# jungmannlab/picasso

Measured on AMD Instinct MI355X. Metric: localizations/sec (7x7 ROI, MLE), higher is better.
Workload: dtype f32+f64; 1 GPU; 10000-frame 512x512 uint16 simulated DNA-PAINT movie per GPU, 1001675 spots per GPU, 7x7 ROI MLE (sigmaxy), identify+cut+fit+table resident in HBM; frames=10000, height=512, width=512, box=7, max_it=100, localizations_total=1001675, mle_mode=refit, refit_spots_rank0=7346, frame_ranges_in_flight=2, all_gather=none

## Files before the change

### picasso_amd/csrc/fit_common.h

```cpp
#pragma once
#include <math.h>

#include "pmi_common.h"

namespace pmi {

#ifndef FIT_WAVES_N
#define FIT_WAVES_N 4
#endif
constexpr int FIT_WAVES = FIT_WAVES_N;
constexpr int FIT_NT = FIT_WAVES * PMI_WAVE;
constexpr int FIT_MAXPIX = PMI_MAX_BOX * PMI_MAX_BOX;

struct ConstDiv { float g, r; int fast; };
inline ConstDiv make_const_div(float g)
{
    ConstDiv c;
    c.g = g;
    c.r = (float)(1.0 / (double)g);
    c.fast = (g == g) && fabsf(g) > 1e-15f && fabsf(g) < 1e15f;
    if (g == 1.0f) c.fast = 2;
    return c;
}
__device__ __forceinline__ float div_const(float x, const ConstDiv &c)
{
    if (c.fast == 2) return x;
    const float ax = fabsf(x);
    if (!c.fast || !((ax > 1e-15f && ax < 1e15f) || x == 0.0f)) return x / c.g;
    const float q = x * c.r;
    const float e = __builtin_fmaf(-q, c.g, x);
    return __builtin_fmaf(e, c.r, q);
}
template <int B> __device__ __forceinline__ void div_const_row(float (&v)[B], const ConstDiv &c)
{
    if (c.fast == 2) return;
    unsigned hi = 0u, lo = 0xffffffffu;
#pragma unroll
    for (int i = 0; i < B; i++) {
        const unsigned u = __float_as_uint(v[i]) & 0x7fffffffu;
        hi = u > hi ? u : hi;
        const unsigned w = u - 1u;
        lo = w < lo ? w : lo;
    }
    if (c.fast && hi < 0x58635fa9u && lo >= 0x26901d7du) {
#pragma unroll
        for (int i = 0; i < B; i++) {
            const float q = v[i] * c.r;
            const float e = __builtin_fmaf(-q, c.g, v[i]);
            v[i] = __builtin_fmaf(e, c.r, q);
        }
    } else {
#pragma unroll
        for (int i = 0; i < B; i++) v[i] = v[i] / c.g;
    }
}

struct FitParams {
    const float *spots;
    float *spots_out;
    const void *movie;
    const int32_t *frame, *y, *x;
    int dtype;
    int64_t Y, X;
    float baseline, sensitivity, gain;
    ConstDiv gdiv;
    int64_t N;
    const int64_t *d_n;
    int box;
    int libm_glibc;
    double eps;
    int max_it;
    float *thetas, *crlbs, *loglik;
    int32_t *iterations;
    unsigned long long *queue;
    unsigned *strict_queue;
    int64_t first;
    double *fisher;
    float eps_lo, eps_hi;
    int32_t *flag_list;
    unsigned *flag_count;
    unsigned *flag_reasons;
    const int32_t *final_list;
    const unsigned *final_list_n;
    unsigned char *refit_mark;
    float *ng_io;
    unsigned char *accept;
    int crop_y0, crop_x0, crop_cy, crop_cx;
    double min_ng;
    const int32_t *alist;
    const unsigned *alist_n;
    int32_t *alist_out;
    unsigned *alist_blk_out;
};
enum : unsigned { FLAG_MARGIN = 1u, FLAG_CURVATURE = 2u, FLAG_NARROW = 4u, FLAG_SWING = 8u, FLAG_WILD = 16u, FLAG_SLOW = 32u, FLAG_UNSTABLE = 64u };
constexpr int FLAG_REASONS = 7;
constexpr double FIT_UNSTABLE_LMAX = 1.9;
constexpr int FISHER_STRIDE = 21;
enum { FIT_STAGE_NEWTON = 1, FIT_STAGE_FINAL = 2, FIT_STAGE_INIT_ONLY = 4, FIT_STAGE_ITERATE_ONLY = 8 };
constexpr int FIT_SLOW_ITERATIONS = 64;
#ifndef PMI_MARGIN_GROWTH
#define PMI_MARGIN_GROWTH 0.0625f
#endif
constexpr float FIT_MARGIN_GROWTH = PMI_MARGIN_GROWTH;
constexpr float FIT_NARROW_SIGMA = 0.5f;
constexpr float FIT_WOBBLE_RATIO = 0.9f;
constexpr float FIT_WOBBLE_FLOOR = 1.9073486e-6f;
constexpr int FIT_WOBBLE_RUN = 3;
constexpr int FIT_WOBBLE_LATE = 9;
constexpr float FIT_TOP_FLAG = 16.0f;

template <int CTRL, int ROW_MASK = 0xf>
__device__ __forceinline__ float dpp_f(float v)
// ... 96 lines not shown
```

### picasso_amd/csrc/gaussmle.hip

```cpp
#include <algorithm>
#include <cmath>
#include <cstdlib>
#include <cstring>
#include <vector>

#include "fit_common.h"

namespace pmi {

__device__ __forceinline__ unsigned borderline(float D, int kk, float eps_lo, float eps_hi)
{
    const float wide = fmaxf(1.0f, (float)(kk - 1) * FIT_MARGIN_GROWTH);
    const float epsf = 0.5f * (eps_lo + eps_hi), epsm = 0.5f * (eps_hi - eps_lo) * wide;
    return ((D >= epsf - epsm && D < epsf + epsm) ? FLAG_MARGIN : 0u) | (kk > FIT_SLOW_ITERATIONS ? FLAG_SLOW : 0u);
}
struct StepHistory { float prev, prev2, wprev; int run; };
__device__ __forceinline__ bool wobbles(float st, float value, int kk, StepHistory &h)
{
    const float w = kk >= 3 ? (st - 2.0f * h.prev) + h.prev2 : 0.0f;
    const bool wob = w * h.wprev < 0.0f && fabsf(w) > FIT_WOBBLE_RATIO * fabsf(h.wprev) && fabsf(w) > FIT_WOBBLE_FLOOR * fabsf(value);
    h.run = wob ? h.run + 1 : 0;
    h.wprev = w; h.prev2 = h.prev; h.prev = st;
    return h.run >= FIT_WOBBLE_RUN || (h.run >= 2 && kk >= FIT_WOBBLE_LATE);
}
// ... 562 lines not shown
        if (!strcmp(env, "glibc")) return PMI_LIBM_GLIBC;
        if (!strcmp(env, "device")) return PMI_LIBM_DEVICE;
    }
    return g_mle_libm;
}

int fit_impl(FitParams p, int method, bool from_movie, int range, hipStream_t s)
{
    if (p.box < 3 || p.box > PMI_MAX_BOX || (p.box & 1) == 0) { set_error("box must be odd, 3..%d (got %d)", PMI_MAX_BOX, p.box); return PMI_ERR_ARG; }
    if (method != PMI_MLE_SIGMA && method != PMI_MLE_SIGMAXY) { set_error("Method not available."); return PMI_ERR_ARG; }
    if (p.N < 0) { set_error("negative N"); return PMI_ERR_ARG; }
    if (p.N == 0) return PMI_OK;
    if (p.N > 0x7fffffffLL) { set_error("too many spots for one call"); return PMI_ERR_ARG; }
    const int g_cu_count = device_cu_count();
    const int mode = mle_mode_now();
    const int64_t BATCH = FIT_BATCH;
    const int64_t nb = (p.N + BATCH - 1) / BATCH;
    void *ptr = nullptr, *fptr = nullptr;
    int rc;
    if ((rc = scratch(SCR_FIT, (size_t)nb * 40 + 64, &ptr)) != PMI_OK) return rc;
    const size_t per_batch = (size_t)std::min<int64_t>(p.N, BATCH);
    const size_t acc_blocks = (per_batch + ACC_BLOCK - 1) / ACC_BLOCK + 2;
    if ((rc = scratch(SCR_STAGE_D, per_batch * (FISHER_STRIDE * sizeof(double) + 12 * sizeof(float) + 3 * sizeof(int32_t) + 1) + acc_blocks * sizeof(unsigned) + 32, &fptr)) != PMI_OK) return rc;
    float *state = reinterpret_cast<float *>((char *)fptr + per_batch * FISHER_STRIDE * sizeof(double));
    int32_t *flag_list = reinterpret_cast<int32_t *>(state + per_batch * 12);
    int32_t *unstable_list = flag_list + per_batch;
    int32_t *acc_list = unstable_list + per_batch;
    unsigned *acc_blk = reinterpret_cast<unsigned *>(acc_list + per_batch);
    unsigned char *refit_mark = reinterpret_cast<unsigned char *>(acc_blk + acc_blocks);
    unsigned long long *queues = (unsigned long long *)ptr;
    unsigned *flag_counts = (unsigned *)(queues + 3 * nb);
    unsigned *strict_queues = flag_counts + 2 * nb;
    void *sptr = nullptr;
    if ((rc = scratch(SCR_STATS, 64, &sptr)) != PMI_OK) return rc;
    unsigned *stats = (unsigned *)sptr;
    hipLaunchKernelGGL(zero_words_kernel, dim3(1), dim3(256), 0, s, (unsigned *)ptr, (int)(nb * 10), stats, 16);
    p.flag_reasons = stats + 1;
    p.fisher = (double *)fptr;
    const int libm = mle_libm_now();
    const bool libm_all = libm != PMI_LIBM_DEVICE;
    p.libm_glibc = libm == PMI_LIBM_GLIBC || (libm == PMI_LIBM_AUTO && p.box <= 5);
    static const char *menv = tuning_env("PMI_MLE_MARGIN");
    const double margin = menv ? atof(menv) : g_mle_margin;
    const double ulp = ldexp(1.0, (int)floor(log2(std::max(1.0, p.box / 2.0))) - 23);
    const double margin_abs = std::max(p.eps * margin, 4.0 * ulp);
    p.eps_lo = (float)(p.eps - margin_abs);
    p.eps_hi = (float)(p.eps + margin_abs);
    const int ppl = (p.box * p.box + 63) / 64;
    const int64_t Ntotal = p.N;
    ScopedKernelTimer tm(s, &g_last_times.fit_ms);
    static const bool force_wave_per_spot = tuning_env("PMI_FIT_WAVE_PER_SPOT") != nullptr;
    const bool g8 = !force_wave_per_spot && p.box <= 15;
    float *cut = nullptr;
    static const bool no_keep = tuning_env("PMI_MLE_NO_KEEP") != nullptr;
    if (g8 && from_movie && mode != PMI_MLE_STRICT && !no_keep) {
        void *cptr = nullptr;
        if ((rc = scratch(SCR_STAGE_C, per_batch * (size_t)(p.box * p.box) * sizeof(float), &cptr)) != PMI_OK) return rc;
        cut = (float *)cptr;
    }
    p.spots_out = nullptr;
    if (p.ng_io && !(g8 && from_movie && cut)) { set_error("deferred exact stage outside the row-per-lane fit"); return PMI_ERR_ARG; }
    for (int64_t bi = 0; bi < nb; bi++) {
        p.first = bi * BATCH;
        p.N = std::min<int64_t>(Ntotal, p.first + BATCH);
        p.flag_list = mode == PMI_MLE_REFIT ? flag_list : nullptr;
        p.flag_count = flag_counts + bi;
        p.strict_queue = strict_queues + bi;
        p.refit_mark = mode == PMI_MLE_REFIT ? refit_mark : nullptr;
        if (p.refit_mark && !g8) PMI_HIP(hipMemsetAsync(refit_mark, 0, (size_t)(p.N - p.first), s));
        const int64_t count = p.N - p.first;
        const int64_t blocks = std::min<int64_t>((count + FIT_WAVES - 1) / FIT_WAVES, (int64_t)g_cu_count * 8);
        const dim3 grid((unsigned)std::max<int64_t>(blocks, 1));
        auto wave_per_spot = [&](int stages) {
            p.queue = queues + 3 * bi + (stages == FIT_STAGE_FINAL ? (p.final_list ? 2 : 1) : 0);
            if (method == PMI_MLE_SIGMAXY) {
                if (from_movie) launch_fit_ppl<6, true>(ppl, grid, s, p, stages); else launch_fit_ppl<6, false>(ppl, grid, s, p, stages);
            } else {
                if (from_movie) launch_fit_ppl<5, true>(ppl, grid, s, p, stages); else launch_fit_ppl<5, false>(ppl, grid, s, p, stages);
            }
        };
        if (mode != PMI_MLE_STRICT && g8 && from_movie && cut) {
            FitParams pi = p;
            pi.spots_out = cut;
            launch_fit_g8(pi, method, true, g_cu_count, state, FIT_STAGE_INIT_ONLY, s);
            PMI_HIP(hipGetLastError());
            FitParams q = p;
            q.spots = cut - p.first * (int64_t)(p.box * p.box);
            if (p.ng_io) {
                int32_t *al = nb == 1 && p.alist_out ? p.alist_out : acc_list;
                unsigned *ab = nb == 1 && p.alist_out ? p.alist_blk_out : acc_blk;
                if ((rc = build_accept_list(p.accept, p.first, p.N, p.d_n, ab, al, s)) != PMI_OK) return rc;
                q.alist = al;
                q.alist_n = ab + (count + ACC_BLOCK - 1) / ACC_BLOCK;
            }
            launch_fit_g8(q, method, false, g_cu_count, state, FIT_STAGE_ITERATE_ONLY, s);
            PMI_HIP(hipGetLastError());
            if (mode == PMI_MLE_REFIT)
                launch_fit_strict(q, method, false, flag_list, q.flag_count, count, g_cu_count, s);
            PMI_HIP(hipGetLastError());
            launch_fit_g8(q, method, false, g_cu_count, state, FIT_STAGE_FINAL, s);
        } else {
        if (mode == PMI_MLE_STRICT) {
            FitParams ps = p;
            ps.libm_glibc = libm_all;
            launch_fit_strict(ps, method, from_movie, nullptr, nullptr, count, g_cu_count, s);
        } else {
            if (g8) launch_fit_g8(p, method, from_movie, g_cu_count, state, FIT_STAGE_NEWTON, s);
            else wave_per_spot(FIT_STAGE_NEWTON);
            PMI_HIP(hipGetLastError());
            if (mode == PMI_MLE_REFIT)
                launch_fit_strict(p, method, from_movie, flag_list, p.flag_count, count, g_cu_count, s);
        }
        PMI_HIP(hipGetLastError());
        if (g8) launch_fit_g8(p, method, from_movie, g_cu_count, state, FIT_STAGE_FINAL, s);
        else wave_per_spot(FIT_STAGE_FINAL);
        }
        PMI_HIP(hipGetLastError());
        const unsigned cb = (unsigned)((count + 255) / 256);
        unsigned *unstable_n = flag_counts + nb + bi;
        auto crlb = [&](const int32_t *list, const unsigned *list_n, int32_t *out, unsigned *out_n) {
            if (method == PMI_MLE_SIGMAXY)
                hipLaunchKernelGGL((crlb_kernel<6>), dim3(cb), dim3(256), 0, s, p.fisher, p.first, p.N, p.d_n, p.crlbs, list, list_n, out, out_n, p.flag_reasons, p.refit_mark, p.accept);
            else
                hipLaunchKernelGGL((crlb_kernel<5>), dim3(cb), dim3(256), 0, s, p.fisher, p.first, p.N, p.d_n, p.crlbs, list, list_n, out, out_n, p.flag_reasons, p.refit_mark, p.accept);
        };
        const bool second = mode == PMI_MLE_REFIT;
        crlb(nullptr, nullptr, second ? unstable_list : nullptr, second ? unstable_n : nullptr);
        PMI_HIP(hipGetLastError());
        if (second) {
            FitParams r = p;
            r.strict_queue = strict_queues + nb + bi;
            if (cut) { r.spots = cut - p.first * (int64_t)(p.box * p.box); }
            const bool r_movie = cut ? false : from_movie;
            launch_fit_strict(r, method, r_movie, unstable_list, unstable_n, count, g_cu_count, s);
            PMI_HIP(hipGetLastError());
            r.final_list = unstable_list; r.final_list_n = unstable_n;
            if (g8) launch_fit_g8(r, method, r_movie, g_cu_count, state, FIT_STAGE_FINAL, s);
            else {
                FitParams keep = p;
                p = r;
                wave_per_spot(FIT_STAGE_FINAL);
                p = keep;
            }
            PMI_HIP(hipGetLastError());
            crlb(unstable_list, unstable_n, nullptr, nullptr);
            PMI_HIP(hipGetLastError());
        }
    }
    hipLaunchKernelGGL(flag_stats_kernel, dim3(1), dim3(1), 0, s, flag_counts, mode == PMI_MLE_REFIT ? 2 * nb : 0, stats);
    PMI_HIP(hipGetLastError());
    if ((rc = g_mle_stats.record(0, range, stats, s)) != PMI_OK) return rc;
    tm.stop();
    return PMI_OK;
}

static int read_last_stats(unsigned (&h)[16], hipStream_t s)
{
    if (g_mle_stats.valid()) PMI_HIP(hipStreamSynchronize(s));
    return g_mle_stats.read(h);
}

__global__ void cut_spots_kernel(const void *__restrict__ movie, int dtype, int64_t Y, int64_t X,
                                 const int32_t *__restrict__ frame, const int32_t *__restrict__ y,
                                 const int32_t *__restrict__ x, int64_t N, const int64_t *__restrict__ d_n,
                                 int box, float baseline, float sensitivity, ConstDiv gdiv, float *__restrict__ spots)
{
    int64_t n = N;
    if (d_n) { int64_t dn = *d_n; n = dn < n ? dn : n; }
    const int npix = box * box, h = box / 2;
    int64_t total = n * npix;
    for (int64_t t = (int64_t)blockIdx.x * blockDim.x + threadIdx.x; t < total; t += (int64_t)gridDim.x * blockDim.x) {
        int64_t i = t / npix;
        int q = (int)(t - i * npix);
        int a = q / box, c = q - a * box;
        float raw = load_movie_px(movie, dtype, ((int64_t)frame[i] * Y + (y[i] - h + a)) * X + (x[i] - h + c));
        spots[t] = div_const((raw - baseline) * sensitivity, gdiv);
    }
}

struct LocCols { void *c[PMI_LOC_COLUMNS]; };
__global__ void locs_from_fits_kernel(const int32_t *__restrict__ frame, const int32_t *__restrict__ y,
                                      const int32_t *__restrict__ x, const float *__restrict__ ng,
                                      const float *__restrict__ th, const float *__restrict__ cr,
                                      const float *__restrict__ ll, const int32_t *__restrict__ it, int64_t N,
                                      const int64_t *__restrict__ d_n, int box, LocCols cols, const int64_t *__restrict__ d_row0,
// ... 319 lines not shown
```

### picasso_amd/csrc/gaussmle_g8.hip

```cpp
#include <algorithm>

#include "fit_common.h"
#include "ng_common.h"

namespace pmi {

__device__ __forceinline__ float sum8(float v)
{
    v += dpp_f<0xB1>(v);
    v += dpp_f<0x4E>(v);
    v += dpp_f<0x141>(v);
    return v;
}
__device__ __forceinline__ float min8(float v)
{
    v = fminf(v, dpp_f<0xB1>(v));
    v = fminf(v, dpp_f<0x4E>(v));
    v = fminf(v, dpp_f<0x141>(v));
    return v;
}
__device__ __forceinline__ double sum8_d(double v)
{
    v += dpp_d<0xB1>(v);
    v += dpp_d<0x4E>(v);
// ... 94 lines not shown
    return t;
}

#ifndef G8_PACKED_BOUNDARY
#define G8_PACKED_BOUNDARY 1
#endif
typedef float f32x2 __attribute__((ext_vector_type(2)));
struct BTerms2 { f32x2 E, A, A2, S, S2; };
__device__ __forceinline__ f32x2 splat2(float v) { return (f32x2){v, v}; }
__device__ __forceinline__ f32x2 fma2(f32x2 a, f32x2 b, f32x2 c) { return __builtin_elementwise_fma(a, b, c); }
__device__ __forceinline__ f32x2 erf_f32x2(f32x2 a)
{
    const f32x2 t = {fabsf(a.x), fabsf(a.y)}, s = a * a;
    f32x2 r = fma2(splat2(-1.72853470e-5f), t, splat2(3.83197126e-4f));
    const f32x2 u = fma2(splat2(-3.88396438e-3f), t, splat2(2.42546219e-2f));
    r = fma2(r, s, u);
    r = fma2(r, t, splat2(-1.06777877e-1f));
    r = fma2(r, t, splat2(-6.34846687e-1f));
    r = fma2(r, t, splat2(-1.28717512e-1f));
    r = fma2(r, t, -t);
    const f32x2 ex = {__expf(r.x), __expf(r.y)};
    const f32x2 one_m = splat2(1.0f) - ex;
    const f32x2 big = {copysignf(one_m.x, a.x), copysignf(one_m.y, a.y)};
    f32x2 q = splat2(-5.96761703e-4f);
    q = fma2(q, s, splat2(4.99119423e-3f));
    q = fma2(q, s, splat2(-2.67681349e-2f));
    q = fma2(q, s, splat2(1.12819925e-1f));
    q = fma2(q, s, splat2(-3.76125336e-1f));
    q = fma2(q, s, splat2(1.28379166e-1f));
    const f32x2 small = fma2(q, a, a);
    return (f32x2){t.x > 0.921875f ? big.x : small.x, t.y > 0.921875f ? big.y : small.y};
}
__device__ __forceinline__ BTerms2 boundary_terms2(float jf, f32x2 mu, f32x2 sigma)
{
    const f32x2 is = {rcp_f32(sigma.x), rcp_f32(sigma.y)};
    const f32x2 sn = splat2(0.70710678118654757f) * is, c1 = splat2(0.3989422804014327f) * is, is2 = is * is;
    const f32x2 u0 = splat2(jf - 0.5f) - mu;
    const f32x2 e0 = erf_f32x2(u0 * sn);
    const f32x2 ga = splat2(-0.5f) * u0 * u0 * is2;
    const f32x2 g0 = {__expf(ga.x), __expf(ga.y)};
    const f32x2 e1 = {from_next(e0.x), from_next(e0.y)}, g1 = {from_next(g0.x), from_next(g0.y)};
    const f32x2 u1 = u0 + splat2(1.0f);
    const f32x2 q1 = u0 * g0 - u1 * g1;
    const f32x2 q3 = u0 * u0 * u0 * g0 - u1 * u1 * u1 * g1;
    BTerms2 t;
    t.E = splat2(0.5f) * (e1 - e0);
    t.A = (g0 - g1) * c1;
    t.A2 = q1 * c1 * is2;
    t.S = q1 * c1 * is;
    t.S2 = c1 * is2 * (q3 * is2 - splat2(2.0f) * q1);
    return t;
}

template <int B, bool FROM_MOVIE>
__device__ __forceinline__ void load_row(const FitParams &p, int64_t sidx, int j, bool valid, float (&d)[B])
{
    constexpr int H = B / 2;
#pragma unroll
    for (int i = 0; i < B; i++) d[i] = 0.f;
    if (valid) {
        if (FROM_MOVIE) {
            float raw[B];
            const int64_t fr = p.frame[sidx], yy = p.y[sidx], xx = p.x[sidx];
            const int64_t o = (fr * p.Y + (yy - H + j)) * p.X + (xx - H);
            switch (p.dtype) {
            case PMI_U16: { const uint16_t *q = (const uint16_t *)p.movie + o; _Pragma("unroll") for (int i = 0; i < B; i++) raw[i] = (float)q[i]; } break;
            case PMI_U8:  { const uint8_t *q = (const uint8_t *)p.movie + o;   _Pragma("unroll") for (int i = 0; i < B; i++) raw[i] = (float)q[i]; } break;
            case PMI_I16: { const int16_t *q = (const int16_t *)p.movie + o;   _Pragma("unroll") for (int i = 0; i < B; i++) raw[i] = (float)q[i]; } break;
            case PMI_U32: { const uint32_t *q = (const uint32_t *)p.movie + o; _Pragma("unroll") for (int i = 0; i < B; i++) raw[i] = (float)q[i]; } break;
            case PMI_I32: { const int32_t *q = (const int32_t *)p.movie + o;   _Pragma("unroll") for (int i = 0; i < B; i++) raw[i] = (float)q[i]; } break;
            default:      { const float *q = (const float *)p.movie + o;       _Pragma("unroll") for (int i = 0; i < B; i++) raw[i] = q[i]; } break;
            }
#pragma unroll
            for (int i = 0; i < B; i++)
                d[i] = (raw[i] - p.baseline) * p.sensitivity;
            div_const_row<B>(d, p.gdiv);
        } else {
            const float *sp = p.spots + sidx * (B * B) + j * B;
#pragma unroll
            for (int i = 0; i < B; i++) d[i] = sp[i];
        }
    }
}

#ifndef G8_REFILL_K
#define G8_REFILL_K 2
#endif
template <int GS> struct GLds { static constexpr int N = GS * 12 + GS * 12 + (GS == 8 ? 16 : 16); };

struct LaneRole {
    float ms;
    float floor_, cap;
    float th;
    float prev, prev2;
    float wprev;
    int run;
    bool conv_rel;
};

template <int NP, int B>
__device__ __forceinline__ bool newton_step(const float (&d)[B], float (&th)[6], LaneRole &role, float *lds,
                                            int j, bool rowok, bool active, int &kk, double eps, int max_it,
                                            float eps_lo, float eps_hi, unsigned &flags)
{
    constexpr int GS = GroupOf<B>::GS;
    float *cols = lds, *red = lds + GS * 12, *bc = lds + 2 * GS * 12;
    const float jf = (float)j;
    const float sgy = NP == 6 ? th[5] : th[4];
    BTerms tx, ty;
#if G8_PACKED_BOUNDARY
    {
        const BTerms2 b = boundary_terms2(jf, (f32x2){th[0], th[1]}, (f32x2){th[4], sgy});
        tx.E = b.E.x; tx.A = b.A.x; tx.A2 = b.A2.x; tx.S = b.S.x; tx.S2 = b.S2.x;
        ty.E = b.E.y; ty.A = b.A.y; ty.A2 = b.A2.y; ty.S = b.S.y; ty.S2 = b.S2.y;
    }
#else
    tx = boundary_terms(jf, th[0], th[4]);
    ty = boundary_terms(jf, th[1], sgy);
#endif
    __builtin_amdgcn_wave_barrier();
    {
        float4 *c = reinterpret_cast<float4 *>(cols + j * 12);
        c[0] = make_float4(tx.A, tx.E, tx.S, tx.A2);
        c[1] = make_float4(tx.S2, 1.0f, tx.A * tx.A, tx.E * tx.E);
        c[2] = make_float4(tx.S * tx.S, 1.0f, tx.S * tx.E, 0.0f);
    }
    __builtin_amdgcn_wave_barrier();
    __threadfence_block();

// ... 201 lines not shown
            if (spot_ok && (rowok || edge_lane)) load_nb_row<W>(p.movie, p.dtype, (fr * p.Y + r1) * p.X + (xx - H - 1), c0, nb);
            if (spot_ok && edge_lane) load_nb_row<W>(p.movie, p.dtype, (fr * p.Y + (yy + H + 1)) * p.X + (xx - H - 1), c0, nb2);
#pragma unroll
            for (int i = 0; i < B; i++) d[i] = 0.f;
            if (spot_ok && rowok) {
#pragma unroll
                for (int i = 0; i < B; i++) d[i] = (nb[i + 1] - p.baseline) * p.sensitivity;
                div_const_row<B>(d, p.gdiv);
            }
            loaded = true;
            if (__any(need)) {
                if (rowok) {
#pragma unroll
                    for (int c = 0; c < W; c++) nbt[(j + 1) * W + c] = nb[c];
                }
                if (edge_lane) {
#pragma unroll
                    for (int c = 0; c < W; c++) { nbt[c] = nb[c]; nbt[(W - 1) * W + c] = nb2[c]; }
                }
                __builtin_amdgcn_wave_barrier();
                __threadfence_block();
                const float vc = nbt[(H + 1) * W + (H + 1)];
                bool fm = true;
                if (rowok) {
#pragma unroll
                    for (int l = 0; l < B; l++) {
                        const float o = nb[l + 1];
                        const bool before = j < H || (j == H && l < H);
                        const bool centre = j == H && l == H;
                        fm = fm && (centre || (before ? vc > o : vc >= o));
                        const float gy = sub_rn(nbt[(j + 2) * W + l + 1], nbt[j * W + l + 1]);
                        const float gx = sub_rn(nb[l + 2], nb[l]);
                        terms[j * B + l] = add_rn(mul_rn(gy, uy[l]), mul_rn(gx, ux[l]));
                    }
                }
                __builtin_amdgcn_wave_barrier();
                __threadfence_block();
                float ng = 0.0f;
#pragma unroll
                for (int q = 0; q < B * B; q++)
                    if (q != H * B + H) ng = add_rn(ng, terms[q]);
                const unsigned long long gm = (GS == 64 ? ~0ull : ((1ull << GS) - 1ull)) << (lane & ~(GS - 1));
                const bool first_max = (__ballot(fm) & gm) == gm;
                if (need) {
                    keep = first_max && (double)ng > p.min_ng;
                    if (j == 0) p.ng_io[sidx] = ng;
                }
                __builtin_amdgcn_wave_barrier();
            }
            if (spot_ok && j == 0) p.accept[sidx] = keep ? 1 : 0;
        }
    }
    if (!loaded) load_row<B, FROM_MOVIE>(p, sidx, j, spot_ok && rowok, d);
    if (FROM_MOVIE && p.spots_out && spot_ok && rowok && keep) {
        float *o = p.spots_out + (sidx - p.first) * (B * B) + j * B;
#pragma unroll
        for (int i = 0; i < B; i++) o[i] = d[i];
    }

    double ps = 0.0, px = 0.0;
#pragma unroll
    for (int i = 0; i < B; i++) { ps += (double)d[i]; px += (double)d[i] * (double)i; }
    double sum = gsum_d<GS>(ps), sx_ = gsum_d<GS>(px), sy_ = gsum_d<GS>(ps * (double)j);
    float fmin_l = INFINITY;
    {
        double t3[B];
#pragma unroll
        for (int i = 0; i < B; i++) {
            double a = (double)d[i];
            if (i > 0) a = (double)d[i - 1] + a;
            if (i + 1 < B) a += (double)d[i + 1];
            t3[i] = a;
        }
        const bool up = j > 0, dn = j + 1 < B;
        const int nrow = 1 + (up ? 1 : 0) + (dn ? 1 : 0);
        const double n2 = (double)(nrow * 2), n3 = (double)(nrow * 3);
        const double r2 = 1.0 / n2, r3 = 1.0 / n3;
#pragma unroll
        for (int i = 0; i < B; i++) {
            const double a = from_prev_d(t3[i]), c = from_next_d(t3[i]);
            double tot = t3[i];
            if (up) tot = a + tot;
            if (dn) tot += c;
            const bool edge = (i == 0) || (i + 1 == B);
            const double nn = edge ? n2 : n3, rr = edge ? r2 : r3;
            double q = tot * rr;
            q = fma(fma(-q, nn, tot), rr, q);
            const float filt = (float)q;
            if (rowok) fmin_l = fminf(fmin_l, filt);
        }
    }
    const float bg0 = (sum != sum) ? (float)sum : gmin<GS>(fmin_l);
    double com_y, com_x;
    if (sum <= 0.0) { sum = 0.01; com_y = (B - 1) / 2.0; com_x = (B - 1) / 2.0; }
    else { com_y = sy_ / sum; com_x = sx_ / sum; }
    double photons = sum - (double)(B * B) * (double)bg0;
    photons = (photons != photons) ? photons : (photons > 1.0 ? photons : 1.0);
    double a_sdy = 0.0, a_sy = 0.0, a_sdx = 0.0, a_sx = 0.0;
    if (rowok) {
        const float vm = d[H] - bg0;
        a_sdy = (double)vm * (double)((j - H) * (j - H));
        a_sy = (double)vm;
        if (j == H) {
#pragma unroll
            for (int i = 0; i < B; i++) {
                const float v2 = d[i] - bg0;
                a_sdx += (double)v2 * (double)((i - H) * (i - H));
                a_sx += (double)v2;
            }
        }
    }
    a_sdy = gsum_d<GS>(a_sdy); a_sy = gsum_d<GS>(a_sy); a_sdx = gsum_d<GS>(a_sdx); a_sx = gsum_d<GS>(a_sx);
    double isy = sqrt(a_sdy / a_sy), isx = sqrt(a_sdx / a_sx);
    if (!isfinite(isy)) isy = 0.01;
    if (!isfinite(isx)) isx = 0.01;
    if (isx == 0) isx = 0.01;
    if (isy == 0) isy = 0.01;

    float th[6], ms[6];
    th[0] = (float)com_x; th[1] = (float)com_y; th[2] = (float)photons; th[3] = bg0;
    if (NP == 6) { th[4] = (float)isx; th[5] = (float)isy; }
    else { th[4] = (float)((isx + isy) / 2); th[5] = 0.f; }
    ms[0] = th[4]; ms[1] = th[4];
    ms[2] = (float)(0.1 * (double)th[2]); ms[3] = (float)(0.1 * (double)th[3]);
    ms[4] = (float)(0.2 * (double)th[4]); ms[5] = (float)(0.2 * (double)th[5]);
    if (spot_ok && j == 0) {
        if (p.refit_mark) p.refit_mark[sidx - p.first] = 0;
        float4 *so = reinterpret_cast<float4 *>(state + (sidx - p.first) * 12);
        so[0] = make_float4(th[0], th[1], th[2], th[3]);
        so[1] = make_float4(th[4], th[5], ms[0], ms[1]);
        so[2] = make_float4(ms[2], ms[3], ms[4], ms[5]);
    }
}

template <int NP, int B, bool FROM_MOVIE>
__global__ __launch_bounds__(FIT_NT) void g8_iterate_kernel(FitParams p, const float *__restrict__ state)
{
    constexpr int GS = GroupOf<B>::GS, NSPW = 64 / GS;
    constexpr int REFILL_K = GS == 8 ? G8_REFILL_K : 1;
    __shared__ __attribute__((aligned(16))) float s_x[FIT_WAVES][NSPW][GLds<GS>::N];
    const int lane = threadIdx.x & 63, wid = threadIdx.x >> 6;
    const int g = lane / GS, j = lane & (GS - 1);
    const bool rowok = j < B;
    int64_t n = p.N;
    if (p.d_n) { int64_t dn = *p.d_n; n = dn < n ? dn : n; }
    const int64_t count = p.alist ? (int64_t)*p.alist_n : n - p.first;
    if (count <= 0) return;
    const int64_t total_waves = (int64_t)gridDim.x * FIT_WAVES;
    const int64_t chunk = (count + total_waves - 1) / total_waves;
    const int64_t wv = (int64_t)blockIdx.x * FIT_WAVES + __builtin_amdgcn_readfirstlane(wid);
    const int64_t base = p.alist ? 0 : p.first, lim = base + count;
    int64_t next = base + wv * chunk;
    const int64_t end = next + chunk < lim ? next + chunk : lim;
    if (next >= end) return;

    float *xs = &s_x[wid][g][0];
    float d[B], th[6], ms[6];
#pragma unroll
    for (int i = 0; i < B; i++) d[i] = 1.f;
#pragma unroll
    for (int l = 0; l < 6; l++) { th[l] = 1.f; ms[l] = 1.f; }
    LaneRole role = make_role<NP, B>(th, ms, j);
    int kk = 0;
    int64_t sidx = -1;
    bool active = false;
    unsigned flags = 0u;
    const unsigned long long below = (1ull << (lane & ~(GS - 1))) - 1ull;

    for (;;) {
        const unsigned long long pend = __ballot(!active && sidx >= 0 && j == 0);
        const unsigned long long empty = __ballot(!active && sidx < 0 && j == 0);
        const bool any_active = __any(active);
        if (__popcll(pend) >= REFILL_K || (pend != 0 && !any_active) || (empty != 0 && next < end)) {
            const unsigned gflag = gor_u<GS>(flags);
            if (!active && sidx >= 0 && j == 0) {
                float *to = p.thetas + sidx * 6;
#pragma unroll
                for (int l = 0; l < 5; l++) to[l] = th[l];
                to[5] = NP == 6 ? th[5] : th[4];
                p.iterations[sidx] = kk;
                if (gflag && p.flag_list) {
                    p.flag_list[atomicAdd(p.flag_count, 1u)] = (int32_t)sidx;
                    count_flag_reasons(p.flag_reasons, gflag);
                }
            }
            const unsigned long long want = pend | empty;
            const int64_t cand = next + __popcll(want & below);
            if (!active) {
                sidx = -1;
                if (cand < end) {
                    sidx = p.alist ? (int64_t)p.alist[cand] : cand;
                    const float4 *si = reinterpret_cast<const float4 *>(state + (sidx - p.first) * 12);
                    const float4 s0 = si[0], s1 = si[1], s2 = si[2];
                    th[0] = s0.x; th[1] = s0.y; th[2] = s0.z; th[3] = s0.w; th[4] = s1.x; th[5] = s1.y;
                    ms[0] = s1.z; ms[1] = s1.w; ms[2] = s2.x; ms[3] = s2.y; ms[4] = s2.z; ms[5] = s2.w;
                    load_row<B, FROM_MOVIE>(p, sidx, j, rowok, d);
                    role = make_role<NP, B>(th, ms, j);
                    kk = 0;
                    flags = 0u;
                    active = p.max_it > 0;
                    if (!active && j == 0) {
                        float *to = p.thetas + sidx * 6;
#pragma unroll
                        for (int l = 0; l < 5; l++) to[l] = th[l];
                        to[5] = NP == 6 ? th[5] : th[4];
                        p.iterations[sidx] = 0;
                        sidx = -1;
                    }
                }
            }
            next += __popcll(want);
            if (!__any(active)) {
                if (next >= end) break;
                continue;
            }
        } else if (!any_active) {
            break;
        }
        active = newton_step<NP, B>(d, th, role, xs, j, rowok, active, kk, p.eps, p.max_it, p.eps_lo, p.eps_hi, flags);
    }
}

template <int NP, int B, bool FROM_MOVIE>
__global__ __launch_bounds__(FIT_NT) void g8_final_kernel(FitParams p)
{
    constexpr int GS = GroupOf<B>::GS, NSPW = 64 / GS;
    __shared__ __attribute__((aligned(16))) double s_x[FIT_WAVES][NSPW][GS * 7];
    const int lane = threadIdx.x & 63, wid = threadIdx.x >> 6;
    const int g = lane / GS, j = lane & (GS - 1);
    const bool rowok = j < B;
    const float jf = (float)j;
    int64_t n = p.N;
    if (p.d_n) { int64_t dn = *p.d_n; n = dn < n ? dn : n; }
    int64_t sidx = p.first + ((int64_t)blockIdx.x * FIT_WAVES + wid) * NSPW + g;
    bool spot_ok = sidx < n;
    if (p.final_list) {
        const int64_t w0 = ((int64_t)blockIdx.x * FIT_WAVES + wid) * NSPW, items = (int64_t)*p.final_list_n;
        if (__builtin_amdgcn_readfirstlane((int)(w0 >= items))) return;
        spot_ok = w0 + g < items;
        sidx = spot_ok ? (int64_t)p.final_list[w0 + g] : p.first;
    } else if (__builtin_amdgcn_readfirstlane((int)(p.first + ((int64_t)blockIdx.x * FIT_WAVES + wid) * NSPW >= n))) return;
    else if (p.accept) spot_ok = spot_ok && p.accept[sidx] != 0;

    float d[B], th[6];
    load_row<B, FROM_MOVIE>(p, sidx, j, spot_ok && rowok, d);
#pragma unroll
    for (int l = 0; l < 6; l++) th[l] = spot_ok ? p.thetas[sidx * 6 + l] : 1.f;
    double *red = &s_x[wid][g][0];
    float *cols = reinterpret_cast<float *>(red);
    const float sgy = NP == 6 ? th[5] : th[4];
    const BTerms tx = boundary_terms<true>(jf, th[0], th[4]);
    const BTerms ty = boundary_terms<true>(jf, th[1], sgy);
    {
        float4 *c = reinterpret_cast<float4 *>(cols + j * 12);
        c[0] = make_float4(tx.A * tx.A, tx.A * tx.E, tx.A, tx.A * tx.S);
        c[1] = make_float4(tx.E * tx.E, tx.E, tx.E * tx.S, 1.0f);
        c[2] = make_float4(tx.S, tx.S * tx.S, 0.f, 0.f);
    }
    __builtin_amdgcn_wave_barrier();
    __threadfence_block();
    double T[10];
#pragma unroll
    for (int e = 0; e < 10; e++) T[e] = 0.0;
    float ll_loc = 0.f;
    const float N_ = th[2];
    const float NEy = N_ * ty.E;
#pragma unroll
    for (int i = 0; i < B; i++) {
        const float4 *c = reinterpret_cast<const float4 *>(cols + i * 12);
        const float4 c0 = c[0], c1 = c[1];
        const float2 c2 = *reinterpret_cast<const float2 *>(cols + i * 12 + 8);
        const float model = NEy * c1.y + th[3];
        if (rowok) {
            const double md = (double)model;
            double inv = (double)rcp_f32(model);
            inv = inv * (2.0 - md * inv);
            inv = inv * (2.0 - md * inv);
            T[0] += (double)c0.x * inv; T[1] += (double)c0.y * inv; T[2] += (double)c0.z * inv; T[3] += (double)c0.w * inv;
            T[4] += (double)c1.x * inv; T[5] += (double)c1.y * inv; T[6] += (double)c1.z * inv; T[7] += inv;
            T[8] += (double)c2.x * inv; T[9] += (double)c2.y * inv;
            if (model > 0.f) {
                if (d[i] > 0.f) ll_loc += d[i] * __logf(model / d[i]) - (model - d[i]);
                else ll_loc += -model;
            }
        }
    }
    __builtin_amdgcn_wave_barrier();
    const double rNE = (double)NEy, rNA = (double)(N_ * ty.A), rE = (double)ty.E, rNS = (double)(N_ * ty.S);
    double Mloc[21];
#pragma unroll
    for (int e = 0; e < 21; e++) Mloc[e] = 0.0;
    if (NP == 6) {
        Mloc[0] = rNE * rNE * T[0];  Mloc[1] = rNE * rNA * T[1];  Mloc[2] = rNE * rE * T[1];   Mloc[3] = rNE * T[2];
        Mloc[4] = rNE * rNE * T[3];  Mloc[5] = rNE * rNS * T[1];
        Mloc[6] = rNA * rNA * T[4];  Mloc[7] = rNA * rE * T[4];   Mloc[8] = rNA * T[5];        Mloc[9] = rNA * rNE * T[6];
        Mloc[10] = rNA * rNS * T[4];
        Mloc[11] = rE * rE * T[4];   Mloc[12] = rE * T[5];        Mloc[13] = rE * rNE * T[6];  Mloc[14] = rE * rNS * T[4];
        Mloc[15] = T[7];             Mloc[16] = rNE * T[8];       Mloc[17] = rNS * T[5];
        Mloc[18] = rNE * rNE * T[9]; Mloc[19] = rNE * rNS * T[6];
        Mloc[20] = rNS * rNS * T[4];
    } else {
        Mloc[0] = rNE * rNE * T[0];  Mloc[1] = rNE * rNA * T[1];  Mloc[2] = rNE * rE * T[1];   Mloc[3] = rNE * T[2];
        Mloc[4] = rNE * (rNE * T[3] + rNS * T[1]);
        Mloc[5] = rNA * rNA * T[4];  Mloc[6] = rNA * rE * T[4];   Mloc[7] = rNA * T[5];
        Mloc[8] = rNA * (rNE * T[6] + rNS * T[4]);
        Mloc[9] = rE * rE * T[4];    Mloc[10] = rE * T[5];        Mloc[11] = rE * (rNE * T[6] + rNS * T[4]);
        Mloc[12] = T[7];             Mloc[13] = rNE * T[8] + rNS * T[5];
        Mloc[14] = rNE * rNE * T[9] + 2.0 * rNE * rNS * T[6] + rNS * rNS * T[4];
    }
    constexpr int NE_ = NP * (NP + 1) / 2;
    double mine[3] = {0.0, 0.0, 0.0};
#pragma unroll
    for (int r0 = 0; r0 < 21; r0 += 7) {
        if (r0 < NE_) {
#pragma unroll
            for (int e = 0; e < 7; e++) red[j * 7 + e] = Mloc[r0 + e];
            __builtin_amdgcn_wave_barrier();
            __threadfence_block();
#pragma unroll
            for (int t = 0; t < 3; t++) {
                const int e = j + GS * t - r0;
                if (e >= 0 && e < 7) {
                    double acc = 0.0;
#pragma unroll
                    for (int r = 0; r < B; r++) acc += red[r * 7 + e];
                    mine[t] = acc;
                }
            }
            __builtin_amdgcn_wave_barrier();
        }
    }
    double *fo = p.fisher + (sidx - p.first) * FISHER_STRIDE;
    if (spot_ok) {
#pragma unroll
        for (int t = 0; t < 3; t++)
            if (j + GS * t < NE_) fo[j + GS * t] = mine[t];
    }
    const float ll = gsum<GS>(ll_loc);
    if (spot_ok && j == 0) p.loglik[sidx] = ll;
}

template <int NP, int B, bool FROM_MOVIE>
static void launch_g8(const FitParams &p, float *state, int cu_count, int stages, hipStream_t s)
{
    constexpr int NSPW = 64 / GroupOf<B>::GS;
    const int64_t count = p.N - p.first;
    const int64_t waves = (count + NSPW - 1) / NSPW;
    const dim3 flat((unsigned)((waves + FIT_WAVES - 1) / FIT_WAVES));
    const int64_t pw = std::max<int64_t>(1, std::min<int64_t>((int64_t)cu_count * 24, (count + 63) / 64));
    const dim3 pers((unsigned)((pw + FIT_WAVES - 1) / FIT_WAVES));
    if (stages & (FIT_STAGE_NEWTON | FIT_STAGE_INIT_ONLY))
        hipLaunchKernelGGL((g8_init_kernel<NP, B, FROM_MOVIE>), flat, dim3(FIT_NT), 0, s, p, state);
    if (stages & (FIT_STAGE_NEWTON | FIT_STAGE_ITERATE_ONLY))
        hipLaunchKernelGGL((g8_iterate_kernel<NP, B, FROM_MOVIE>), pers, dim3(FIT_NT), 0, s, p, (const float *)state);
    if (stages & FIT_STAGE_FINAL)
        hipLaunchKernelGGL((g8_final_kernel<NP, B, FROM_MOVIE>), flat, dim3(FIT_NT), 0, s, p);
}

template <int NP, bool FROM_MOVIE>
static void launch_g8_box(const FitParams &p, float *state, int cu_count, int stages, hipStream_t s)
{
    switch (p.box) {
    case 3: launch_g8<NP, 3, FROM_MOVIE>(p, state, cu_count, stages, s); break;
    case 5: launch_g8<NP, 5, FROM_MOVIE>(p, state, cu_count, stages, s); break;
    case 7: launch_g8<NP, 7, FROM_MOVIE>(p, state, cu_count, stages, s); break;
    case 9: launch_g8<NP, 9, FROM_MOVIE>(p, state, cu_count, stages, s); break;
    case 11: launch_g8<NP, 11, FROM_MOVIE>(p, state, cu_count, stages, s); break;
    case 13: launch_g8<NP, 13, FROM_MOVIE>(p, state, cu_count, stages, s); break;
    default: launch_g8<NP, 15, FROM_MOVIE>(p, state, cu_count, stages, s); break;
    }
}

bool launch_fit_g8(const FitParams &p, int method, bool from_movie, int cu_count, float *state, int stages, hipStream_t s)
{
    if (p.box > 15) return false;
    if (method == PMI_MLE_SIGMAXY) {
        if (from_movie) launch_g8_box<6, true>(p, state, cu_count, stages, s); else launch_g8_box<6, false>(p, state, cu_count, stages, s);
    } else {
        if (from_movie) launch_g8_box<5, true>(p, state, cu_count, stages, s); else launch_g8_box<5, false>(p, state, cu_count, stages, s);
    }
    return true;
}

}
```

### picasso_amd/csrc/gaussmle_strict.hip

```cpp
#include <algorithm>
#include <cstdlib>

#include "fit_common.h"

#pragma clang fp contract(off)

#include "libm_glibc.h"

namespace pmi {

namespace {

__constant__ uint64_t k_glibc_exp_tab[PMI_GLIBC_EXP_TABLE_WORDS] = {
#include "libm_glibc_exp_table.inc"
};

typedef double d2_t __attribute__((ext_vector_type(2)));
constexpr double K_SQRT_2PI = 2.5066282746310002;
constexpr double K_SQRT_2 = 1.4142135623730951;
constexpr double K_SQRT_PI = 1.7724538509055159;

__device__ __forceinline__ double np_max_d(double a, double b) { return (a != a) ? a : ((b != b) ? b : (a > b ? a : b)); }
__device__ __forceinline__ double np_min_d(double a, double b) { return (a != a) ? a : ((b != b) ? b : (a < b ? a : b)); }
__device__ __forceinline__ float div_rn(float a, float b) { return (float)((double)a / (double)b); }

__device__ __forceinline__ double shared_div(double n, double d, double r)
{
    double q = n * r;
    double e = __builtin_fma(-q, d, n);
    q = __builtin_fma(e, r, q);
    e = __builtin_fma(-q, d, n);
    return __builtin_fma(e, r, q);
}
__device__ __forceinline__ bool mid_or_zero(double v)
{
    const unsigned e = ((unsigned)__double2hiint(v) >> 20) & 0x7ffu;
    return (e - 823u) < 400u || v == 0.0;
}

__device__ __forceinline__ void lds_sync()
{
    __builtin_amdgcn_wave_barrier();
    __threadfence_block();
    __builtin_amdgcn_wave_barrier();
}

template <int GS> struct SLds {
    static constexpr int MAXB = GS == 16 ? 7 : (GS == 32 ? 15 : PMI_MAX_BOX);
    static constexpr int SPOT = ((MAXB * MAXB * 4 + 15) / 16) * 16;
    static constexpr int BS = 2 * (MAXB + 1);
    static constexpr int CS = 2 * MAXB;
    static constexpr int RS = GS + (GS == 16 ? 4 : 2);
    static constexpr int BND = 4 * BS * 8;
    static constexpr int COL = 5 * CS * 8;
    static constexpr int TERM = 12 * RS * 8;
    static constexpr int ACC = 24 * 4;
    static constexpr int BYTES = SPOT + BND + COL + TERM + ACC;
    static constexpr int PAIR_PAD = GS == 16 ? 112 : 0;
    static constexpr int NSPW = 64 / GS;
    static constexpr int WAVE_BYTES = NSPW * BYTES + (NSPW / 2) * PAIR_PAD;
    static_assert(BYTES % 16 == 0 && PAIR_PAD % 16 == 0 && (BS * 8) % 16 == 0 && (CS * 8) % 16 == 0 && (RS * 8) % 16 == 0, "LDS layout of a group");
    static_assert(GS != 16 || (BYTES + PAIR_PAD) % 256 == 80, "the chain lanes of a pair of groups share a ds_read_b128: rows 0..3 of one beside rows 4..11 of the other");
    static_assert(3 * ((FIT_WAVES * WAVE_BYTES + 4 + 1279) / 1280) * 1280 <= 160 * 1024, "three workgroups per CU");
};

}

template <int GS, bool FROM_MOVIE>
__device__ __forceinline__ void strict_load_spot(const FitParams &p, int64_t sidx, bool have, int j, float *spot)
{
    const int B = p.box, npix = B * B, H = B / 2;
    int64_t base = 0;
    if (FROM_MOVIE && have) base = (p.frame[sidx] * p.Y + (p.y[sidx] - H)) * p.X + (p.x[sidx] - H);
    for (int q0 = j; q0 < npix; q0 += 8 * GS) {
        float v[8];
#pragma unroll
        for (int u = 0; u < 8; u++) {
            const int q = q0 + u * GS;
            v[u] = 0.f;
            if (have && q < npix) {
                if (FROM_MOVIE) {
                    const int a = q / B, c = q - a * B;
                    v[u] = load_movie_px(p.movie, p.dtype, base + (int64_t)a * p.X + c);
                } else {
                    v[u] = p.spots[sidx * npix + q];
                }
            }
        }
#pragma unroll
        for (int u = 0; u < 8; u++) {
            const int q = q0 + u * GS;
            if (q < npix) spot[q] = (FROM_MOVIE && have) ? div_const((v[u] - p.baseline) * p.sensitivity, p.gdiv) : v[u];
        }
    }
    lds_sync();
}

template <int NP, int GS>
__device__ __forceinline__ void strict_start_values(int B, int j, const float *spot, float *fscr, float (&th)[6])
{
    const int npix = B * B, H = B / 2;
    float best = INFINITY;
    for (int q = j; q < npix; q += GS) {
        const int k = q / B, l = q - k * B;
        const int m0 = k - 1 > 0 ? k - 1 : 0, m1 = k + 2 < B ? k + 2 : B;
        const int n0 = l - 1 > 0 ? l - 1 : 0, n1 = l + 2 < B ? l + 2 : B;
        double nsum = 0.0;
        for (int m = m0; m < m1; m++)
            for (int c = n0; c < n1; c++) nsum += (double)spot[m * B + c];
        const float f = (float)(nsum / (double)((m1 - m0) * (n1 - n0)));
        best = (best != best) ? best : ((f != f) ? f : (f < best ? f : best));
    }
    fscr[j] = best;
    lds_sync();
    float bg0 = INFINITY;
    for (int r = 0; r < GS; r++) {
        const float f = fscr[r];
        bg0 = (bg0 != bg0) ? bg0 : ((f != f) ? f : (f < bg0 ? f : bg0));
    }
    double s_ = 0.0, sy_ = 0.0, sx_ = 0.0;
    for (int a = 0; a < B; a++)
        for (int c = 0; c < B; c++) {
            const double v = (double)spot[a * B + c];
            sy_ += v * (double)a;
            sx_ += v * (double)c;
            s_ += v;
// ... 417 lines not shown
```

Measured before the change: 374.4 million localizations/s.

## Pack cut pixels and initial fit state into one 64-float spot record

For boxes up to 7, the init kernel now writes each spot's cut pixels into a padded 8x8 record, along with theta and max-step in the spare row and column, in place of separate cut and state buffers. The iterate, final and strict kernels read pixels and state from that record with aligned float4 loads. In the iterate kernel, the next spot's record is fetched before the previous result is published, so the load latency can overlap the stores. The record is larger than a 7x7 cut, so more scratch memory is used and more bytes are written for each spot.

```diff
diff --git a/picasso_amd/csrc/fit_common.h b/picasso_amd/csrc/fit_common.h
--- a/picasso_amd/csrc/fit_common.h
+++ b/picasso_amd/csrc/fit_common.h
@@ -2,6 +2,7 @@
 #include <math.h>
 
 #include "pmi_common.h"
+#include "spot_record.h"
 
 namespace pmi {
 
@@ -58,6 +59,7 @@
 struct FitParams {
     const float *spots;
     float *spots_out;
+    int rec;
     const void *movie;
     const int32_t *frame, *y, *x;
     int dtype;
diff --git a/picasso_amd/csrc/gaussmle.hip b/picasso_amd/csrc/gaussmle.hip
--- a/picasso_amd/csrc/gaussmle.hip
+++ b/picasso_amd/csrc/gaussmle.hip
@@ -638,13 +638,16 @@
     static const bool force_wave_per_spot = tuning_env("PMI_FIT_WAVE_PER_SPOT") != nullptr;
     const bool g8 = !force_wave_per_spot && p.box <= 15;
     float *cut = nullptr;
+    const bool cut_rec = p.box <= rec::MAX_BOX;
+    const int64_t cut_stride = cut_rec ? rec::FLOATS : p.box * p.box;
     static const bool no_keep = tuning_env("PMI_MLE_NO_KEEP") != nullptr;
     if (g8 && from_movie && mode != PMI_MLE_STRICT && !no_keep) {
         void *cptr = nullptr;
-        if ((rc = scratch(SCR_STAGE_C, per_batch * (size_t)(p.box * p.box) * sizeof(float), &cptr)) != PMI_OK) return rc;
+        if ((rc = scratch(SCR_STAGE_C, per_batch * (size_t)cut_stride * sizeof(float), &cptr)) != PMI_OK) return rc;
         cut = (float *)cptr;
     }
     p.spots_out = nullptr;
+    p.rec = 0;
     if (p.ng_io && !(g8 && from_movie && cut)) { set_error("deferred exact stage outside the row-per-lane fit"); return PMI_ERR_ARG; }
     for (int64_t bi = 0; bi < nb; bi++) {
         p.first = bi * BATCH;
@@ -671,7 +674,8 @@
             launch_fit_g8(pi, method, true, g_cu_count, state, FIT_STAGE_INIT_ONLY, s);
             PMI_HIP(hipGetLastError());
             FitParams q = p;
-            q.spots = cut - p.first * (int64_t)(p.box * p.box);
+            q.spots = cut - p.first * cut_stride;
+            q.rec = cut_rec ? 1 : 0;
             if (p.ng_io) {
                 int32_t *al = nb == 1 && p.alist_out ? p.alist_out : acc_list;
                 unsigned *ab = nb == 1 && p.alist_out ? p.alist_blk_out : acc_blk;
@@ -716,7 +720,7 @@
         if (second) {
             FitParams r = p;
             r.strict_queue = strict_queues + nb + bi;
-            if (cut) { r.spots = cut - p.first * (int64_t)(p.box * p.box); }
+            if (cut) { r.spots = cut - p.first * cut_stride; r.rec = cut_rec ? 1 : 0; }
             const bool r_movie = cut ? false : from_movie;
             launch_fit_strict(r, method, r_movie, unstable_list, unstable_n, count, g_cu_count, s);
             PMI_HIP(hipGetLastError());
diff --git a/picasso_amd/csrc/gaussmle_g8.hip b/picasso_amd/csrc/gaussmle_g8.hip
--- a/picasso_amd/csrc/gaussmle_g8.hip
+++ b/picasso_amd/csrc/gaussmle_g8.hip
@@ -170,7 +170,7 @@
     return t;
 }
 
-template <int B, bool FROM_MOVIE>
+template <int B, bool FROM_MOVIE, bool REC = false>
 __device__ __forceinline__ void load_row(const FitParams &p, int64_t sidx, int j, bool valid, float (&d)[B])
 {
     constexpr int H = B / 2;
@@ -193,6 +193,12 @@
             for (int i = 0; i < B; i++)
                 d[i] = (raw[i] - p.baseline) * p.sensitivity;
             div_const_row<B>(d, p.gdiv);
+        } else if (REC) {
+            const float4 *rp = reinterpret_cast<const float4 *>(p.spots + sidx * rec::FLOATS + rec::pixel(j, 0));
+            const float4 a = rp[0], b = rp[1];
+            const float v[8] = {a.x, a.y, a.z, a.w, b.x, b.y, b.z, b.w};
+#pragma unroll
+            for (int i = 0; i < B; i++) d[i] = v[i];
         } else {
             const float *sp = p.spots + sidx * (B * B) + j * B;
 #pragma unroll
@@ -500,7 +506,8 @@
         }
     }
     if (!loaded) load_row<B, FROM_MOVIE>(p, sidx, j, spot_ok && rowok, d);
-    if (FROM_MOVIE && p.spots_out && spot_ok && rowok && keep) {
+    constexpr bool RECORD = FROM_MOVIE && B <= rec::MAX_BOX;
+    if (FROM_MOVIE && !RECORD && p.spots_out && spot_ok && rowok && keep) {
         float *o = p.spots_out + (sidx - p.first) * (B * B) + j * B;
 #pragma unroll
         for (int i = 0; i < B; i++) o[i] = d[i];
@@ -572,8 +579,31 @@
     ms[0] = th[4]; ms[1] = th[4];
     ms[2] = (float)(0.1 * (double)th[2]); ms[3] = (float)(0.1 * (double)th[3]);
     ms[4] = (float)(0.2 * (double)th[4]); ms[5] = (float)(0.2 * (double)th[5]);
-    if (spot_ok && j == 0) {
-        if (p.refit_mark) p.refit_mark[sidx - p.first] = 0;
+    if (spot_ok && j == 0 && p.refit_mark) p.refit_mark[sidx - p.first] = 0;
+    if (RECORD && p.spots_out) {
+        static_assert(!RECORD || (GS == 8 && rec::STATE_ROW == GS - 1 && rec::theta(0) % 4 == 0 && rec::pixel(1, 0) % 4 == 0), "record layout");
+        if (spot_ok && keep) {
+            float *r = p.spots_out + (sidx - p.first) * rec::FLOATS;
+            float ms_own = 0.f;
+#pragma unroll
+            for (int l = 2; l < 6; l++) ms_own = (j == l) ? ms[l] : ms_own;
+            if (j == rec::STATE_ROW) {
+                float4 *so = reinterpret_cast<float4 *>(r + rec::theta(0));
+                so[0] = make_float4(th[0], th[1], th[2], th[3]);
+                so[1] = make_float4(th[4], th[5], ms[0], ms[1]);
+            } else if (B == 7) {
+                float4 *ro = reinterpret_cast<float4 *>(r + rec::pixel(j, 0));
+                ro[0] = make_float4(d[0], d[1], d[2], d[3]);
+                ro[1] = make_float4(d[4 % B], d[5 % B], d[6 % B], ms_own);
+            } else {
+                if (rowok) {
+#pragma unroll
+                    for (int i = 0; i < B; i++) r[rec::pixel(j, i)] = d[i];
+                }
+                if (j >= 2 && j < 6) r[rec::max_step(j)] = ms_own;
+            }
+        }
+    } else if (spot_ok && j == 0) {
         float4 *so = reinterpret_cast<float4 *>(state + (sidx - p.first) * 12);
         so[0] = make_float4(th[0], th[1], th[2], th[3]);
         so[1] = make_float4(th[4], th[5], ms[0], ms[1]);
@@ -581,10 +611,11 @@
     }
 }
 
-template <int NP, int B, bool FROM_MOVIE>
+template <int NP, int B, bool FROM_MOVIE, bool REC = false>
 __global__ __launch_bounds__(FIT_NT) void g8_iterate_kernel(FitParams p, const float *__restrict__ state)
 {
     constexpr int GS = GroupOf<B>::GS, NSPW = 64 / GS;
+    static_assert(!REC || (!FROM_MOVIE && GS == 8 && B <= rec::MAX_BOX), "records: boxes up to 7 of the fused path");
     constexpr int REFILL_K = GS == 8 ? G8_REFILL_K : 1;
     __shared__ __attribute__((aligned(16))) float s_x[FIT_WAVES][NSPW][GLds<GS>::N];
     const int lane = threadIdx.x & 63, wid = threadIdx.x >> 6;
@@ -621,28 +652,54 @@
         const bool any_active = __any(active);
         if (__popcll(pend) >= REFILL_K || (pend != 0 && !any_active) || (empty != 0 && next < end)) {
             const unsigned gflag = gor_u<GS>(flags);
-            if (!active && sidx >= 0 && j == 0) {
-                float *to = p.thetas + sidx * 6;
-#pragma unroll
-                for (int l = 0; l < 5; l++) to[l] = th[l];
-                to[5] = NP == 6 ? th[5] : th[4];
-                p.iterations[sidx] = kk;
+            const unsigned long long want = pend | empty;
+            const int64_t cand = next + __popcll(want & below);
+            const bool take = !active && cand < end;
+            constexpr bool EARLY = NP == 6;
+            const bool publish = !active && sidx >= 0 && j == 0;
+            const int64_t osidx = sidx;
+            const int okk = kk;
+            float oth[6];
+#pragma unroll
+            for (int l = 0; l < 6; l++) oth[l] = th[l];
+            auto fetch_record = [&]() {
+                sidx = p.alist ? (int64_t)p.alist[cand] : cand;
+                const float4 *rp = reinterpret_cast<const float4 *>(p.spots + sidx * rec::FLOATS);
+                const float4 r0 = rp[2 * j], r1 = rp[2 * j + 1];
+                const float4 s0 = rp[rec::theta(0) / 4], s1 = rp[rec::theta(0) / 4 + 1];
+                th[0] = s0.x; th[1] = s0.y; th[2] = s0.z; th[3] = s0.w; th[4] = s1.x; th[5] = s1.y;
+                ms[0] = s1.z; ms[1] = s1.w; ms[2] = r1.w; ms[3] = r1.w; ms[4] = r1.w; ms[5] = r1.w;
+                const float v[8] = {r0.x, r0.y, r0.z, r0.w, r1.x, r1.y, r1.z, r1.w};
+#pragma unroll
+                for (int i = 0; i < B; i++) d[i] = v[i];
+            };
+            if (REC && EARLY && take) fetch_record();
+            if (publish) {
+                float *to = p.thetas + osidx * 6;
+#pragma unroll
+                for (int l = 0; l < 5; l++) to[l] = oth[l];
+                to[5] = NP == 6 ? oth[5] : oth[4];
+                p.iterations[osidx] = okk;
                 if (gflag && p.flag_list) {
-                    p.flag_list[atomicAdd(p.flag_count, 1u)] = (int32_t)sidx;
+                    p.flag_list[atomicAdd(p.flag_count, 1u)] = (int32_t)osidx;
                     count_flag_reasons(p.flag_reasons, gflag);
                 }
             }
-            const unsigned long long want = pend | empty;
-            const int64_t cand = next + __popcll(want & below);
+            if (REC && !EARLY && take) fetch_record();
             if (!active) {
-                sidx = -1;
-                if (cand < end) {
-                    sidx = p.alist ? (int64_t)p.alist[cand] : cand;
-                    const float4 *si = reinterpret_cast<const float4 *>(state + (sidx - p.first) * 12);
-                    const float4 s0 = si[0], s1 = si[1], s2 = si[2];
-                    th[0] = s0.x; th[1] = s0.y; th[2] = s0.z; th[3] = s0.w; th[4] = s1.x; th[5] = s1.y;
-                    ms[0] = s1.z; ms[1] = s1.w; ms[2] = s2.x; ms[3] = s2.y; ms[4] = s2.z; ms[5] = s2.w;
-                    load_row<B, FROM_MOVIE>(p, sidx, j, rowok, d);
+                if (!(REC && take)) sidx = -1;
+                if (take) {
+                    if (REC) {
+#pragma unroll
+                        for (int i = 0; i < B; i++) d[i] = rowok ? d[i] : 0.f;
+                    } else {
+                        sidx = p.alist ? (int64_t)p.alist[cand] : cand;
+                        const float4 *si = reinterpret_cast<const float4 *>(state + (sidx - p.first) * 12);
+                        const float4 t0 = si[0], t1 = si[1], t2 = si[2];
+                        th[0] = t0.x; th[1] = t0.y; th[2] = t0.z; th[3] = t0.w; th[4] = t1.x; th[5] = t1.y;
+                        ms[0] = t1.z; ms[1] = t1.w; ms[2] = t2.x; ms[3] = t2.y; ms[4] = t2.z; ms[5] = t2.w;
+                        load_row<B, FROM_MOVIE>(p, sidx, j, rowok, d);
+                    }
                     role = make_role<NP, B>(th, ms, j);
                     kk = 0;
                     flags = 0u;
@@ -669,7 +726,7 @@
     }
 }
 
-template <int NP, int B, bool FROM_MOVIE>
+template <int NP, int B, bool FROM_MOVIE, bool REC = false>
 __global__ __launch_bounds__(FIT_NT) void g8_final_kernel(FitParams p)
 {
     constexpr int GS = GroupOf<B>::GS, NSPW = 64 / GS;
@@ -691,7 +748,7 @@
     else if (p.accept) spot_ok = spot_ok && p.accept[sidx] != 0;
 
     float d[B], th[6];
-    load_row<B, FROM_MOVIE>(p, sidx, j, spot_ok && rowok, d);
+    load_row<B, FROM_MOVIE, REC>(p, sidx, j, spot_ok && rowok, d);
 #pragma unroll
     for (int l = 0; l < 6; l++) th[l] = spot_ok ? p.thetas[sidx * 6 + l] : 1.f;
     double *red = &s_x[wid][g][0];
@@ -797,6 +854,15 @@
     const dim3 flat((unsigned)((waves + FIT_WAVES - 1) / FIT_WAVES));
     const int64_t pw = std::max<int64_t>(1, std::min<int64_t>((int64_t)cu_count * 24, (count + 63) / 64));
     const dim3 pers((unsigned)((pw + FIT_WAVES - 1) / FIT_WAVES));
+    if constexpr (!FROM_MOVIE && B <= rec::MAX_BOX) {
+        if (p.rec) {
+            if (stages & (FIT_STAGE_NEWTON | FIT_STAGE_ITERATE_ONLY))
+                hipLaunchKernelGGL((g8_iterate_kernel<NP, B, false, true>), pers, dim3(FIT_NT), 0, s, p, (const float *)nullptr);
+            if (stages & FIT_STAGE_FINAL)
+                hipLaunchKernelGGL((g8_final_kernel<NP, B, false, true>), flat, dim3(FIT_NT), 0, s, p);
+            return;
+        }
+    }
     if (stages & (FIT_STAGE_NEWTON | FIT_STAGE_INIT_ONLY))
         hipLaunchKernelGGL((g8_init_kernel<NP, B, FROM_MOVIE>), flat, dim3(FIT_NT), 0, s, p, state);
     if (stages & (FIT_STAGE_NEWTON | FIT_STAGE_ITERATE_ONLY))
diff --git a/picasso_amd/csrc/gaussmle_strict.hip b/picasso_amd/csrc/gaussmle_strict.hip
--- a/picasso_amd/csrc/gaussmle_strict.hip
+++ b/picasso_amd/csrc/gaussmle_strict.hip
@@ -72,6 +72,21 @@
     const int B = p.box, npix = B * B, H = B / 2;
     int64_t base = 0;
     if (FROM_MOVIE && have) base = (p.frame[sidx] * p.Y + (p.y[sidx] - H)) * p.X + (p.x[sidx] - H);
+    if (!FROM_MOVIE && p.rec) {
+        for (int t = j; t < 2 * B; t += GS) {
+            const int a = t >> 1, c0 = (t & 1) * 4;
+            if (c0 < B) {
+                float4 v4 = make_float4(0.f, 0.f, 0.f, 0.f);
+                if (have) v4 = *reinterpret_cast<const float4 *>(p.spots + sidx * rec::FLOATS + rec::pixel(a, c0));
+                const float v[4] = {v4.x, v4.y, v4.z, v4.w};
+#pragma unroll
+                for (int u = 0; u < 4; u++)
+                    if (c0 + u < B) spot[a * B + c0 + u] = v[u];
+            }
+        }
+        lds_sync();
+        return;
+    }
     for (int q0 = j; q0 < npix; q0 += 8 * GS) {
         float v[8];
 #pragma unroll
diff --git a/picasso_amd/csrc/spot_record.h b/picasso_amd/csrc/spot_record.h
--- /dev/null
+++ b/picasso_amd/csrc/spot_record.h
@@ -0,0 +1,16 @@
+#pragma once
+
+namespace pmi {
+namespace rec {
+
+constexpr int FLOATS = 64;
+constexpr int ROW = 8;
+constexpr int MAX_BOX = 7;
+constexpr int STATE_ROW = 7;
+
+constexpr int pixel(int j, int i) { return ROW * j + i; }
+constexpr int theta(int l) { return ROW * STATE_ROW + l; }
+constexpr int max_step(int l) { return l < 2 ? ROW * STATE_ROW + 6 + l : ROW * l + 7; }
+
+}
+}
```

Result: no change. 373.0 million localizations/s (median of 2 runs) (-0.3%).
